# raviraina/grok

Measured on AMD Instinct MI355X. Metric: Mpixels/s encode+decode, 8K RGB 5/3 lossless + 9/7 lossy, 1/2/4/8 GPU, higher is better.
Workload: dtype int32 (5/3) + f32 (9/7)

## Files before the change

grok_amd/csrc/gk_engine.cpp:

```cpp
#include <hip/hip_runtime.h>

#include <algorithm>
#include <array>
#include <tuple>
#include <cmath>
#include <cstdarg>
#include <cstdlib>
#include <cstdio>
#include <cstring>
#include <memory>
#include <string>
#include <atomic>
#include <chrono>
#include <condition_variable>
#include <functional>
#include <mutex>
#include <thread>
#include <unordered_map>
#include <vector>
#include <queue>
#include <map>
#include <climits>
#include <linux/futex.h>
#include <sys/syscall.h>
// ... 3092 lines not shown
                    }
                    ctx->tm.dwt_launches++;
                    ctx->tm.dwt_bytes += area * (4 + es) * nc;
                    c += nc;
                }
                continue;
            }
            const GkComps cs{cst, ncr};
            if (irrev) {
                float* fs = reinterpret_cast<float*>(src_l);
                float* fd = reinterpret_cast<float*>(dst_l);
                if (forward) gk_launch_dwt97_fwd(ctx->st, fs, RG.stride, fd, RG.stride, w, h, S.tb, cs);
                else gk_launch_dwt97_inv(ctx->st, fd, RG.stride, fs, RG.stride, w, h, S.tb, cs);
            } else {
                if (forward) gk_launch_dwt53_fwd(ctx->st, src_l, RG.stride, dst_l, RG.stride, w, h, S.tb, cs);
                else gk_launch_dwt53_inv(ctx->st, dst_l, RG.stride, src_l, RG.stride, w, h, S.tb, cs);
            }
            ctx->tm.dwt_launches++;
            ctx->tm.dwt_bytes += area * 8 * ncr;
        }
    }
    }
}

static float ev_ms(gk_ctx* ctx, int a, int b) {
    float ms = 0; (void)hipEventElapsedTime(&ms, ctx->ev[a], ctx->ev[b]); return ms;
}

static void setup_plan(gk_ctx* ctx, const gk_image_info* info, const gk_cparameters* cp) {
    Plan want;
    want.w = info->w; want.h = info->h; want.nc = info->numcomps; want.prec = info->prec; want.sgnd = info->sgnd;
    set_params(want.p, cp, want.nc);
    want.x0 = info->x0; want.y0 = info->y0;
    want.gx0 = cp ? cp->tx0 : 0; want.gy0 = cp ? cp->ty0 : 0;
    if (!ctx->enc_dx.empty()) {
        if (ctx->enc_dx.size() != want.nc) throw GkError("gk_set_subsampling was given a different component count");
        want.cdx = ctx->enc_dx; want.cdy = ctx->enc_dy;
        if (!want.subsampled()) { want.cdx.clear(); want.cdy.clear(); }
    }
    if (want.gx0 > want.x0 || want.gy0 > want.y0) throw GkError("tile grid origin must lie at or above-left of the image origin");
    if ((uint64_t)want.x0 + want.w > 0xffffffffull || (uint64_t)want.y0 + want.h > 0xffffffffull)
        throw GkError("image area past the 32-bit canvas");
    if (want.p.tw && ((uint64_t)want.gx0 + want.p.tw <= want.x0 || (uint64_t)want.gy0 + want.p.th <= want.y0))
        throw GkError("the first tile must overlap the image area");
    if (want.nc < 3) want.p.mct = 0;
    if (ctx->enc_col.clears_mct()) want.p.mct = 0;
    if (want.p.mct && !want.mct3()) want.p.mct = 0;
    check_poc_coverage(want.p, want.nc);
    if ((want.p.cblk_sty & GK_STY_HT) && want.p.cblk_sty != GK_STY_HT)
        throw GkError("HTJ2K cannot be combined with Part-1 mode switches");
    if (want.p.cblk_sty > 0x7f) throw GkError("unknown code-block style bits");
    if (want.nc > 255 || want.nc == 0) throw GkError("bad component count");
    if (want.prec == 0 || want.prec > 31) throw GkError("component precision must be 1..31 bits");
    check_precision(want);
    if (want.w == 0 || want.h == 0) throw GkError("empty image");
    if (want.p.jp2) ctx->enc_jp2h = jp2h_content(want, &ctx->enc_col);
    if (want.p.cbw < 2 || want.p.cbh < 2 || want.p.cbw > 10 || want.p.cbh > 10 || want.p.cbw + want.p.cbh > 12)
        throw GkError("code-block size must be 4..1024 per side with at most 4096 samples");
    ensure_plan(ctx, want);
    restore_native_qcd(ctx);
    if (!ctx->plan.p.roishift.empty())
    for (const TileG& T : ctx->plan.tiles)
        for (uint32_t ci = 0; ci < (uint32_t)T.comps.size(); ++ci)
            for (const ResG& R : T.comps[ci].res)
                for (const auto& B : R.bands)
                    if (ctx->plan.p.roi(ci) && B.numbps > 25) throw GkError("ROI shift too large for this precision");
}

static void dump_blocks(gk_ctx* ctx, const uint32_t* hinfo, const GkPass* dps, uint32_t npass_total,
                        uint8_t* dbytes, uint64_t slot0) {
    const Plan& P = ctx->plan;
    hipStream_t st = ctx->st;
    const bool ht = P.p.ht();
    std::vector<GkPass> hp(std::max(npass_total, 1u));
    if (!ht && npass_total)
        HIPCHK(hipMemcpyAsync(hp.data(), dps, sizeof(GkPass) * npass_total, hipMemcpyDeviceToHost, st));
    HIPCHK(hipStreamSynchronize(st));
    ctx->rb_bands.clear(); ctx->rb_blocks.clear(); ctx->rb_passes.clear();
    std::vector<uint64_t> seg;
    uint64_t pos = 0;
    const TileG& T = P.tiles[0];
    for (uint32_t c = 0; c < P.nc; ++c)
        for (uint32_t r = 0; r < P.p.numres; ++r) {
            const ResG& R = T.comps[c].res[r];
            for (uint32_t bi = 0; bi < R.bands.size(); ++bi) {
                const BandG& B = R.bands[bi];
                ctx->rb_bands.push_back({c, r, bi, B.orient, R.pw * R.ph, B.step_enc});
                for (uint32_t pi = 0; pi < R.pw * R.ph; ++pi) {
                    const PrecG& PG = R.prc[bi][pi];
                    for (uint32_t k = 0; k < PG.cw * PG.ch; ++k) {
                        const uint32_t b = PG.first_block + k;
                        const GkBlock& G = P.blocks[b];
                        gk_block_result o{};
                        o.comp = c; o.res = r; o.band = bi; o.precinct = pi; o.cblk = k;
                        o.x0 = P.bxy[2 * (size_t)b]; o.y0 = P.bxy[2 * (size_t)b + 1];
                        o.x1 = o.x0 + G.w; o.y1 = o.y0 + G.h;
                        o.numbps = hinfo[4 * (size_t)b]; o.npasses = hinfo[4 * (size_t)b + 1];
                        o.len = hinfo[4 * (size_t)b + 2];
                        o.pass_off = (uint32_t)ctx->rb_passes.size();
                        o.data_off = pos;
                        const uint64_t so = G.data_off - slot0;
                        if (ht && o.npasses) {
                            const uint32_t ms = hinfo[4 * (size_t)b + 3], tl = o.len - ms;
                            if (ms) { seg.push_back(so); seg.push_back(pos); seg.push_back(ms); }
                            seg.push_back(so + G.data_cap - tl); seg.push_back(pos + ms); seg.push_back(tl);
                            ctx->rb_passes.push_back({o.len, o.len, 0.0});
                        } else if (o.npasses) {
                            seg.push_back(so); seg.push_back(pos); seg.push_back(o.len);
                            const GkPass* ps = hp.data() + hinfo[4 * (size_t)b + 3];
                            for (uint32_t q = 0; q < o.npasses; ++q)
                                ctx->rb_passes.push_back({q + 1 == o.npasses ? o.len : ps[q].rate, ps[q].len, ps[q].dist});
                        }
                        pos += o.len;
                        ctx->rb_blocks.push_back(o);
                    }
                }
            }
        }
    ctx->rb_data.resize(pos);
    if (pos) {
        uint64_t* hs = (uint64_t*)ctx->hseg.get(seg.size() * 8);
        memcpy(hs, seg.data(), seg.size() * 8);
        uint64_t* ds = (uint64_t*)ctx->dseg.get(seg.size() * 8);
        HIPCHK(hipMemcpyAsync(ds, hs, seg.size() * 8, hipMemcpyHostToDevice, st));
        uint8_t* dst = (uint8_t*)ctx->dout.get(pos);
        gk_launch_gather(st, dbytes, dst, ds, (uint32_t)(seg.size() / 3));
        HIPCHK(hipMemcpyAsync(ctx->rb_data.data(), dst, pos, hipMemcpyDeviceToHost, st));
        HIPCHK(hipStreamSynchronize(st));
    }
}

struct PixSrc { const void* pixels; size_t row_bytes; int on_device; };

static size_t encode_impl(gk_ctx* ctx, const gk_image_info* info, const void* const* comps, const uint32_t* strides,
                          int comps_on_device, const gk_cparameters* cp, uint8_t* out, size_t cap, int out_on_device,
                          int* rc, uint32_t tb = 0, uint32_t te = 0, bool with_header = true,
                          uint32_t* part_lens = nullptr, bool blocks_only = false, const PixSrc* pix = nullptr) {
    setup_plan(ctx, info, cp);
    Plan& P = ctx->plan;
    const uint32_t ntiles = (uint32_t)P.tiles.size();
    if (te == 0) { tb = 0; te = ntiles; }
    if (tb >= te || te > ntiles) throw GkError("bad tile range");
    const bool sub = P.subsampled();
    const uint32_t nb = (uint32_t)P.blocks.size();
    const uint32_t b0 = P.tiles[tb].b0, b1 = P.tiles[te - 1].b1, nbr = b1 - b0;
    const uint32_t jb = tb / P.ntx, je = (te - 1) / P.ntx + 1;
    const uint32_t ry0 = P.tiles[jb * P.ntx].y0 - P.y0, ry1 = P.tiles[(je - 1) * P.ntx].y1 - P.y0;
    hipStream_t st = ctx->st;

    launch_check(__LINE__);

    HIPCHK(hipEventRecord(ctx->ev[0], st));
    const Region RG = make_region(0, ry0, P.w, ry1);
    int32_t* arena = (int32_t*)ctx->arena.get(RG.plane * P.nc * 2 * sizeof(int32_t));
    const uint32_t nrows = ry1 - ry0;
    const int stype = sample_type(info->sample_bytes, P.prec, P.sgnd != 0);
    const size_t es = gk_sample_size(stype);
    std::vector<const void*> src(P.nc);
    std::vector<uint32_t> sstr(P.nc);
    std::vector<Region> RGg;
    for (const SGroup& G : P.groups) RGg.push_back(group_region(P, RG, G));
    if (pix) {
        const size_t tight = (size_t)RG.w * P.nc * es;
        const uint8_t* first = (const uint8_t*)pix->pixels + (size_t)RG.y0 * pix->row_bytes;
        GkUnpixArgs ua{};
        ua.ds = align_up(RG.w, GK_UNPIX_ALIGN);
        ua.plane = (uint64_t)ua.ds * RG.h;
        ua.w = RG.w; ua.h = RG.h; ua.nch = P.nc;
        ua.dst = ctx->dplanes.get(ua.plane * P.nc * es);
        ua.src = first; ua.row_bytes = pix->row_bytes;
        if (!pix->on_device) {
            void* dp = ctx->dpix_in.get(tight * RG.h);
            HIPCHK(hipMemcpy2DAsync(dp, tight, first, pix->row_bytes, tight, RG.h, hipMemcpyHostToDevice, st));
            ua.src = dp; ua.row_bytes = tight;
        }
        gk_launch_unpixels(st, (int)es, ua);
        for (uint32_t c = 0; c < P.nc; ++c) { src[c] = (const uint8_t*)ua.dst + (size_t)c * ua.plane * es; sstr[c] = ua.ds; }
    } else {
        size_t tot = 0;
        for (uint32_t c = 0; c < P.nc; ++c) tot += (size_t)RGg[P.group_of[c]].w * RGg[P.group_of[c]].h;
        uint8_t* dp = comps_on_device ? nullptr : (uint8_t*)ctx->dplanes.get(tot * es + 16);
        size_t o = 0;
        for (uint32_t c = 0; c < P.nc; ++c) {
            const Region& R = RGg[P.group_of[c]];
            const uint8_t* first = (const uint8_t*)comps[c] + (size_t)R.y0 * strides[c] * es;
            if (comps_on_device) { src[c] = first; sstr[c] = strides[c]; continue; }
            HIPCHK(hipMemcpy2DAsync(dp + o * es, (size_t)R.w * es, first, (size_t)strides[c] * es, (size_t)R.w * es, R.h,
                                    hipMemcpyHostToDevice, st));
            src[c] = dp + o * es; sstr[c] = R.w;
            o += (size_t)R.w * R.h;
        }
    }
    launch_check(__LINE__);
    HIPCHK(hipEventRecord(ctx->ev[1], st));
    int32_t shift = P.sgnd ? 0 : (1 << (P.prec - 1));
    auto planeA = [&](uint32_t c) { return arena + (size_t)c * 2 * RG.plane; };
    auto planeAf = [&](uint32_t c) { return reinterpret_cast<float*>(planeA(c)); };
    const bool mct3 = P.mct3();
    if (mct3 && (sstr[1] != sstr[0] || sstr[2] != sstr[0])) throw GkError("the first three components must share a stride");
    L1Io io;
    const bool fused = P.p.numres > 1 && P.l1_fusable;
    if (fused) {
        io.stype = stype; io.mct3 = mct3; io.shift.assign(P.nc, shift);
        io.planes.assign(src.begin(), src.end());
        io.strides = sstr;
    } else {
        auto cw = [&](uint32_t c) { return RGg[P.group_of[c]].w; };
        auto ch = [&](uint32_t c) { return RGg[P.group_of[c]].h; };
        if (!P.p.irrev) {
            if (mct3) gk_launch_dc_rct_fwd(st, stype, src[0], src[1], src[2], sstr[0], planeA(0), planeA(1), planeA(2), RG.stride, cw(0), ch(0), shift);
            for (uint32_t c = mct3 ? 3 : 0; c < P.nc; ++c) gk_launch_dc_fwd(st, stype, src[c], sstr[c], planeA(c), RG.stride, cw(c), ch(c), shift);
        } else {
            if (mct3) gk_launch_dc_ict_fwd(st, stype, src[0], src[1], src[2], sstr[0], planeAf(0), planeAf(1), planeAf(2), RG.stride, cw(0), ch(0), shift);
            for (uint32_t c = mct3 ? 3 : 0; c < P.nc; ++c) gk_launch_dc_fwd_f(st, stype, src[c], sstr[c], planeAf(c), RG.stride, cw(c), ch(c), shift);
        }
    }
    launch_check(__LINE__);
    HIPCHK(hipEventRecord(ctx->ev[2], st));
    run_dwt(ctx, RG, true, jb, je, 0, 0xffffffffu, fused ? &io : nullptr);
    if (const char* dp = getenv("GK_DUMP_DWT")) {
        std::vector<int32_t> hv((size_t)P.nc * 2 * RG.plane);
        HIPCHK(hipMemcpyAsync(hv.data(), arena, hv.size() * 4, hipMemcpyDeviceToHost, st));
        HIPCHK(hipStreamSynchronize(st));
        if (FILE* f = fopen(dp, "wb")) {
            const uint32_t hd[4] = {P.nc, RG.stride, RG.h, RG.w};
            fwrite(hd, 4, 4, f);
            fwrite(hv.data(), 4, hv.size(), f);
            fclose(f);
        }
    }
    launch_check(__LINE__);
    HIPCHK(hipEventRecord(ctx->ev[3], st));
    const bool do_rc = P.p.rate_control();
    const uint64_t slot0 = P.blocks[b0].data_off;
    const uint64_t slot1 = b1 < nb ? P.blocks[b1].data_off : P.slot_bytes;
    const uint64_t slot_span = slot1 - slot0;
    uint8_t* dbytes = (uint8_t*)ctx->bytes.get(slot_span + (64u << 20));
    const uint32_t nbx = std::max(nbr, 1u);
    GkBlock* dblk = (GkBlock*)ctx->dblocks.get(sizeof(GkBlock) * nbx);
    GkPass* dps = (GkPass*)ctx->dpasses.get(sizeof(GkPass) * GK_MAX_PASSES * (size_t)nbx);
    uint32_t* dinfo = (uint32_t*)ctx->dinfo.get(16 * (size_t)nbx + 16);
    int* derr = (int*)ctx->derr.get(64);
    uint32_t* dpcount = (uint32_t*)(derr + 4);
    uint8_t* dsym = P.p.ht() ? nullptr : (uint8_t*)ctx->dsym.get(P.sym_off[b1] - P.sym_off[b0] + 256);
    uint64_t* dsymoff = (uint64_t*)ctx->dsymoff.get(8 * ((size_t)nbr + 1));
    uint32_t* dpe = (uint32_t*)ctx->dpassend.get(4 * GK_MAX_PASSES * (size_t)nbx);
    uint32_t* dcm = (uint32_t*)ctx->dcminfo.get(8 * (size_t)nbx);
    int32_t* dnmse = do_rc ? (int32_t*)ctx->dnmse.get(4 * GK_MAX_PASSES * (size_t)nbx) : nullptr;
    if (!ctx->blocks_uploaded || ctx->enc_b0 != b0 || ctx->enc_b1 != b1 || ctx->enc_rc != do_rc) {
        GkBlock* hb = (GkBlock*)ctx->hpasses.get(sizeof(GkBlock) * nbx + 8 * ((size_t)nbr + 1));
        uint64_t* hso = (uint64_t*)(hb + nbx);
        for (uint32_t i = 0; i < nbr; ++i) {
            hb[i] = P.blocks[b0 + i];
            hb[i].band_off = relocate(P, group_region(P, RG, P.groups[P.group_of[hb[i].comp]]), hb[i].band_off);
            hb[i].stride = RG.stride;
            hb[i].data_off -= slot0;
            hb[i].flags = (uint8_t)((hb[i].flags & ~2u) | (do_rc ? 2u : 0u));
        }
        for (uint32_t i = 0; i <= nbr; ++i) hso[i] = P.sym_off[b0 + i] - P.sym_off[b0];
        HIPCHK(hipMemcpyAsync(dblk, hb, sizeof(GkBlock) * nbr, hipMemcpyHostToDevice, st));
        HIPCHK(hipMemcpyAsync(dsymoff, hso, 8 * ((size_t)nbr + 1), hipMemcpyHostToDevice, st));
        HIPCHK(hipStreamSynchronize(st));
        ctx->blocks_uploaded = true; ctx->enc_b0 = b0; ctx->enc_b1 = b1; ctx->enc_rc = do_rc;
    }
    HIPCHK(hipMemsetAsync(derr, 0, 64, st));
    const uint32_t nsolo_env = []() { const char* v = getenv("GK_T1ENC_SOLO"); return v ? (uint32_t)atoi(v) : 0u; }();
    if (P.p.ht()) {
        uint8_t* mel = (uint8_t*)ctx->dsym.get((size_t)nbx * GK_HT_MEL_CAP + 256);
        launch_check(__LINE__);
        HIPCHK(hipEventRecord(ctx->ev[8], st));
        gk_launch_ht_enc(st, arena, dblk, dbytes, mel, GK_HT_MEL_CAP, dinfo, nbr, derr, P.p.wide());
    } else if (P.p.t1_generic()) {
        uint8_t* mst = (uint8_t*)ctx->dmsstate.get(gk_t1ms_state_bytes(nbx));
        launch_check(__LINE__);
        HIPCHK(hipEventRecord(ctx->ev[8], st));
        gk_launch_t1_enc_ms(st, arena, dblk, dbytes, dps, dinfo, nbr, derr, ctx->nmse_tab, dpcount, mst, P.p.cblk_sty & 0x3f);
    } else if (nbr < 8192 || getenv("GK_T1ENC_SERIAL")) {
        gk_launch_t1_cm(st, arena, dblk, dsymoff, dsym, dpe, dcm, nbr, derr, ctx->nmse_tab, dnmse);
        launch_check(__LINE__);
        HIPCHK(hipEventRecord(ctx->ev[8], st));
        gk_launch_t1_mq(st, dsym, dsymoff, dpe, dcm, dblk, dbytes, dps, dinfo, nbr, derr, dnmse, dpcount, nullptr, 0,
                        0xffffffffu, std::min(nsolo_env, nbr));
    } else {
        uint32_t* dw = (uint32_t*)ctx->dweight.get(4 * (size_t)nbr);
        gk_launch_t1_weight(st, arena, dblk, dw, nbr);
        uint32_t* hw = (uint32_t*)ctx->hweight.get(4 * (size_t)nbr);
        HIPCHK(hipMemcpyAsync(hw, dw, 4 * (size_t)nbr, hipMemcpyDeviceToHost, st));
        HIPCHK(hipStreamSynchronize(st));
        uint32_t wmax = 1;
        for (uint32_t i = 0; i < nbr; ++i) wmax = std::max(wmax, hw[i]);
        const uint32_t kB = 4096;
        auto key = [&](uint32_t i) { return kB - 1 - (uint32_t)(((uint64_t)hw[i] * (kB - 1)) / wmax); };
        std::vector<uint32_t> start(kB + 1, 0);
        for (uint32_t i = 0; i < nbr; ++i) start[key(i)]++;
        for (uint32_t k = 0, acc = 0; k <= kB; ++k) { const uint32_t c = start[k]; start[k] = acc; acc += c; }
        uint32_t* ho = (uint32_t*)ctx->hord_enc.get(4 * (size_t)nbr);
        for (uint32_t i = 0; i < nbr; ++i) ho[start[key(i)]++] = i;
        uint32_t* dord = (uint32_t*)ctx->dord_enc.get(4 * (size_t)nbr);
        HIPCHK(hipMemcpyAsync(dord, ho, 4 * (size_t)nbr, hipMemcpyHostToDevice, st));
        static std::vector<double> frs[2];
        std::vector<double>& fr = frs[do_rc ? 1 : 0];
        if (fr.empty()) {
            const char* cv = getenv("GK_T1ENC_CUTS");
            std::string cs = cv ? cv : (do_rc ? "0.08,0.25" : "0.125,0.375");
            for (size_t q = 0; q < cs.size();) {
                size_t e = cs.find(',', q);
                if (e == std::string::npos) e = cs.size();
                const double f = atof(cs.substr(q, e - q).c_str());
                if (f > 0 && f < 1 && fr.size() < 3) fr.push_back(f);
                q = e + 1;
            }
        }
        std::vector<uint32_t> cut(1, 0);
        for (double f : fr) {
            const uint32_t c = (uint32_t)(nbr * f) / 256 * 256;
            if (c > cut.back() && c < nbr) cut.push_back(c);
        }
        cut.push_back(nbr);
        const int nch = (int)cut.size() - 1;
        for (int k = 0; k < nch; ++k) {
            const uint32_t base = cut[k], cnt = cut[k + 1] - cut[k];
            gk_launch_t1_cm(st, arena, dblk, dsymoff, dsym, dpe, dcm, nbr, derr, ctx->nmse_tab, dnmse, dord, base, cnt);
            if (k + 1 < nch) {
                HIPCHK(hipEventRecord(ctx->xev[k], st));
                HIPCHK(hipStreamWaitEvent(ctx->aux[k], ctx->xev[k], 0));
                gk_launch_t1_mq(ctx->aux[k], dsym, dsymoff, dpe, dcm, dblk, dbytes, dps, dinfo, nbr, derr, dnmse, dpcount,
                                dord, base, cnt, k == 0 ? std::min(nsolo_env, cnt) : 0u);
                HIPCHK(hipEventRecord(ctx->xev[3 + k], ctx->aux[k]));
            } else {
                launch_check(__LINE__);
                HIPCHK(hipEventRecord(ctx->ev[8], st));
                gk_launch_t1_mq(st, dsym, dsymoff, dpe, dcm, dblk, dbytes, dps, dinfo, nbr, derr, dnmse, dpcount, dord,
                                base, cnt);
            }
        }
        for (int k = 0; k + 1 < nch; ++k) HIPCHK(hipStreamWaitEvent(st, ctx->xev[3 + k], 0));
    }
    launch_check(__LINE__);
    HIPCHK(hipEventRecord(ctx->ev[4], st));
    static const bool eprof = getenv("GK_PROFILE") != nullptr;
    using eclk = std::chrono::steady_clock;
    auto ems = [](eclk::time_point a, eclk::time_point b) { return std::chrono::duration<double, std::milli>(b - a).count(); };
    const auto te0 = eclk::now();
    uint32_t* hinfo = (uint32_t*)ctx->hinfo.get(16 * (size_t)nb + 64);
    HIPCHK(hipMemcpyAsync(hinfo + 4 * (size_t)b0, dinfo, 16 * (size_t)nbr, hipMemcpyDeviceToHost, st));
    HIPCHK(hipMemcpyAsync(hinfo + 4 * (size_t)nb, derr, 32, hipMemcpyDeviceToHost, st));
    HIPCHK(hipStreamSynchronize(st));
    const uint32_t t1err = hinfo[4 * (size_t)nb], npass_total = hinfo[4 * (size_t)nb + 4];
    if (t1err) throw GkError(t1err & 2 ? "T1 symbol buffer overflow" : "T1 code-block slot overflow");
    const bool ht = P.p.ht();
    const GkPass* hpasses = nullptr;
    if ((do_rc || (P.p.cblk_sty & (GK_STY_LAZY | GK_STY_TERMALL))) && !ht) {
        GkPass* hp = (GkPass*)ctx->hpasses.get(sizeof(GkPass) * (size_t)std::max(npass_total, 1u));
        HIPCHK(hipMemcpyAsync(hp, dps, sizeof(GkPass) * (size_t)npass_total, hipMemcpyDeviceToHost, st));
        HIPCHK(hipStreamSynchronize(st));
        hpasses = hp;
    }
    if (blocks_only) {
        dump_blocks(ctx, hinfo, dps, npass_total, dbytes, slot0);
        *rc = 0;
        return 0;
    }

    std::vector<uint8_t> H;
    H.reserve(1 << 12);
    size_t tlm_pos = 0;
    write_main_header(H, P, &tlm_pos);
    const size_t rc_header_size = H.size() + (P.p.jp2 ? jp2_prefix_size(P, ctx->enc_jp2h) : 0);
    if (!with_header) H.clear();
    const auto te1 = eclk::now();
    if (const char* ds = getenv("GK_DUMP_SYMS"); ds && dsym && !P.p.t1_generic()) {
        std::vector<uint32_t> pe((size_t)GK_MAX_PASSES * nbr), cm(2 * (size_t)nbr), out(2 * (size_t)nbr);
        HIPCHK(hipMemcpy(pe.data(), dpe, 4 * pe.size(), hipMemcpyDeviceToHost));
        HIPCHK(hipMemcpy(cm.data(), dcm, 4 * cm.size(), hipMemcpyDeviceToHost));
        for (uint32_t i = 0; i < nbr; ++i) {
            out[2 * i] = cm[2 * i + 1] ? pe[(size_t)GK_MAX_PASSES * i + cm[2 * i + 1] - 1] : 0;
            out[2 * i + 1] = cm[2 * i];
        }
        if (FILE* f = fopen(ds, "wb")) { fwrite(out.data(), 4, out.size(), f); fclose(f); }
    }
    if (const char* dp = getenv("GK_DUMP_PASSES")) {
        if (FILE* f = fopen(dp, "wb")) {
            const uint32_t hdr[2] = {nb, npass_total};
            fwrite(hdr, 4, 2, f);
            fwrite(hinfo, 16, nb, f);
            if (hpasses) fwrite(hpasses, sizeof(GkPass), npass_total, f);
            fclose(f);
        }
    }
    T2Enc T2(P, hinfo, hpasses, tb, te);
    std::vector<T2Enc::Swallow> tsw(te - tb);
    if (te - tb == 1 || !P.p.rate_control()) {
        T2.allocate(rc_header_size);
        tsw[0] = T2.final_sw;
    } else {
        const bool par = te - tb >= host_pool().size();
        auto one = [&](size_t q) {
            const uint32_t t = tb + (uint32_t)q;
            T2Enc Tt(P, hinfo, hpasses, t, t + 1);
            Tt.serial = par;
            Tt.allocate(rc_header_size);
            tsw[q] = Tt.final_sw;
            const TileG& TG = P.tiles[t];
            std::copy(Tt.lnp.begin() + (size_t)TG.b0 * T2.L, Tt.lnp.begin() + (size_t)TG.b1 * T2.L,
                      T2.lnp.begin() + (size_t)TG.b0 * T2.L);
        };
        if (par) host_pool().run(te - tb, one);
        else for (uint32_t q = 0; q < te - tb; ++q) one(q);
    }
    const auto te2 = eclk::now();
    std::vector<uint64_t> seg;
    seg.reserve(3 * ((size_t)nb * (ht ? 2 : 1) + 64));
    std::vector<uint8_t> hdrs;
    uint64_t pos = 0;
    auto add_host = [&](const uint8_t* p, size_t n) {
        if (!n) return;
        seg.push_back(slot_span + hdrs.size()); seg.push_back(pos); seg.push_back(n);
        hdrs.insert(hdrs.end(), p, p + n);
        pos += n;
    };
    std::vector<uint8_t> J;
    const bool jp2 = P.p.jp2 && with_header;
    if (jp2) write_jp2_prefix(J, P, 0, ctx->enc_jp2h);
    add_host(J.data(), J.size());
    const size_t main_at = J.size();
    add_host(H.data(), H.size());
    struct Pk { uint32_t hoff, hlen, s0, s1, len; };
    struct TileOut {
        std::vector<uint8_t> tp;
        std::vector<uint8_t> phdr;
        std::vector<Pk> pk;
        std::vector<uint32_t> bsegs;
        uint64_t psot = 0;
        std::vector<uint32_t> pkey;
        std::vector<uint32_t> tp_off, pk_first;
        std::vector<uint64_t> psots;
    };
    const TilePartSplit TPS = tile_part_split(P);
    if (part_lens && TPS.n > 1) throw GkError("tile-part generation is not supported with tile sharding");
    std::vector<TileOut> tout(te - tb);
    const bool par_chains = te - tb == 1;
    auto build_tile_part = [&](uint32_t t, TileOut& O) {
        const TileG& T = P.tiles[t];
        const T2Enc::Swallow& sw = tsw[t - tb];
        struct Chain { uint32_t r, c, pi; };
        std::vector<Chain> chains;
        for (uint32_t r = 0; r < P.p.numres; ++r)
            for (uint32_t c = 0; c < P.nc; ++c)
                for (uint32_t pi = 0; pi < T.comps[c].res[r].pw * T.comps[c].res[r].ph; ++pi) chains.push_back({r, c, pi});
        const uint32_t L = P.p.nlayers;
        std::vector<TileOut> co(chains.size());
        auto run_chain = [&](size_t q) {
            const Chain& ch = chains[q];
            const ResG& R = T.comps[ch.c].res[ch.r];
            TileOut& C = co[q];
            std::vector<uint32_t> body;
            std::vector<uint8_t> hb;
            for (uint32_t l = 0; l < L; ++l) {
                body.clear();
                T2.write_packet(R, ch.pi, l, nullptr, &body, hb);
                Pk k{(uint32_t)C.phdr.size(), (uint32_t)hb.size(), (uint32_t)C.bsegs.size(), 0, (uint32_t)hb.size()};
                C.phdr.insert(C.phdr.end(), hb.begin(), hb.end());
                for (size_t i = 0; i < body.size(); i += 3) {
                    if (!body[i + 2]) continue;
                    C.bsegs.push_back(body[i]); C.bsegs.push_back(body[i + 1]); C.bsegs.push_back(body[i + 2]);
                    k.len += body[i + 2];
                }
                k.s1 = (uint32_t)C.bsegs.size();
                C.pk.push_back(k);
            }
        };
        if (par_chains && chains.size() > 1) {
            struct BandU { uint32_t q, bi; };
            std::vector<BandU> bu;
            std::vector<uint32_t> bu0(chains.size() + 1, 0);
            for (size_t q = 0; q < chains.size(); ++q) {
                const ResG& R = T.comps[chains[q].c].res[chains[q].r];
                for (uint32_t bi = 0; bi < R.bands.size(); ++bi)
                    if (R.prc[bi][chains[q].pi].cw && R.prc[bi][chains[q].pi].ch) bu.push_back({(uint32_t)q, bi});
                bu0[q + 1] = (uint32_t)bu.size();
            }
            std::vector<std::vector<RawBits>> ubit(bu.size(), std::vector<RawBits>(L));
            std::vector<std::vector<uint32_t>> useg(bu.size());
            std::vector<std::vector<uint32_t>> uend(bu.size(), std::vector<uint32_t>(L));
            std::vector<size_t> bord(bu.size());
            for (size_t i = 0; i < bord.size(); ++i) bord[i] = bord.size() - 1 - i;
            host_pool().run(bord.size(), [&](size_t j) {
                const size_t u = bord[j];
                const Chain& ch = chains[bu[u].q];
                const ResG& R = T.comps[ch.c].res[ch.r];
                const PrecG& PG = R.prc[bu[u].bi][ch.pi];
                T2.band_init(PG, R.bands[bu[u].bi].numbps);
                std::vector<uint32_t>& sg = useg[u];
                for (uint32_t l = 0; l < L; ++l) {
                    RawBits& rb = ubit[u][l];
                    T2.band_header(PG, l, rb);
                    rb.finish();
                    for (uint32_t k = 0; k < PG.cw * PG.ch; ++k) {
                        const uint32_t b = PG.first_block + k;
                        const uint32_t np = T2.lnp[(size_t)b * L + l];
                        if (!np) continue;
                        const uint32_t r0 = T2.inprev[b] ? T2.rate(b, T2.inprev[b] - 1) : 0, r1 = T2.rate(b, T2.inprev[b] + np - 1);
                        if (r1 > r0) { sg.push_back(b); sg.push_back(r0); sg.push_back(r1 - r0); }
                        T2.inprev[b] = (uint16_t)(T2.inprev[b] + np);
                    }
                    uend[u][l] = (uint32_t)sg.size();
                }
            });
            host_pool().run(chains.size(), [&](size_t q) {
                TileOut& C = co[q];
                for (uint32_t l = 0; l < L; ++l) {
                    const uint32_t h0 = (uint32_t)C.phdr.size();
                    PktBitWriter bw(C.phdr);
                    bw.putbit(1);
                    for (uint32_t u = bu0[q]; u < bu0[q + 1]; ++u) {
                        const RawBits& rb = ubit[u][l];
                        const size_t full = (size_t)(rb.n / 64);
                        const uint32_t rem = (uint32_t)(rb.n % 64);
                        for (size_t i = 0; i < full; ++i) { bw.put((uint32_t)(rb.w[i] >> 32), 32); bw.put((uint32_t)rb.w[i], 32); }
                        if (rem) {
                            const uint64_t x = rb.w[full] >> (64 - rem);
                            if (rem > 32) { bw.put((uint32_t)(x >> 32), rem - 32); bw.put((uint32_t)x, 32); }
                            else bw.put((uint32_t)x, rem);
                        }
                    }
                    bw.flush();
                    const uint32_t hlen = (uint32_t)C.phdr.size() - h0;
                    Pk k{h0, hlen, (uint32_t)C.bsegs.size(), 0, hlen};
                    for (uint32_t u = bu0[q]; u < bu0[q + 1]; ++u) {
                        const uint32_t s0 = l ? uend[u][l - 1] : 0, s1 = uend[u][l];
                        for (uint32_t i = s0; i < s1; i += 3) k.len += useg[u][i + 2];
                        C.bsegs.insert(C.bsegs.end(), useg[u].begin() + s0, useg[u].begin() + s1);
                    }
                    k.s1 = (uint32_t)C.bsegs.size();
                    C.pk.push_back(k);
                }
            });
        } else {
            for (size_t q = 0; q < chains.size(); ++q) run_chain(q);
        }
        std::vector<uint32_t> chain_at(P.p.numres * P.nc + 1, 0);
        for (uint32_t r = 0, q = 0; r < P.p.numres; ++r)
            for (uint32_t c = 0; c < P.nc; ++c) { chain_at[r * P.nc + c] = q; q += T.comps[c].res[r].pw * T.comps[c].res[r].ph; }
        std::vector<uint32_t> entry;
        const std::vector<PacketRef> order = packet_order(P, T, L, &P.p.pocs, TPS.poc ? &entry : nullptr);
        for (size_t oi = 0; oi < order.size(); ++oi) {
                const PacketRef& pr = order[oi];
                O.pkey.push_back(TPS.poc ? entry[2 * oi] : TPS.key(pr));
                const size_t q = chain_at[pr.r * P.nc + pr.c] + pr.pi;
                const uint32_t l = pr.l;
                const TileOut& C = co[q];
                Pk k = C.pk[l];
                const uint32_t h0 = (uint32_t)O.phdr.size(), s0 = (uint32_t)O.bsegs.size();
                if (P.p.sop_eph & 2) {
                    const uint32_t nsop = (TPS.poc ? entry[2 * oi + 1] : (uint32_t)O.pk.size()) & 0xffff;
                    const uint8_t sop[6] = {0xff, 0x91, 0, 4, (uint8_t)(nsop >> 8), (uint8_t)nsop};
                    O.phdr.insert(O.phdr.end(), sop, sop + 6);
                }
                O.phdr.insert(O.phdr.end(), C.phdr.begin() + k.hoff, C.phdr.begin() + k.hoff + k.hlen);
                if (P.p.sop_eph & 4) { O.phdr.push_back(0xff); O.phdr.push_back(0x92); }
                const uint32_t ovh = ((P.p.sop_eph & 2) ? 6 : 0) + ((P.p.sop_eph & 4) ? 2 : 0);
                k.hlen += ovh; k.len += ovh;
                O.bsegs.insert(O.bsegs.end(), C.bsegs.begin() + k.s0, C.bsegs.begin() + k.s1);
                k.hoff = h0; k.s1 = s0 + (k.s1 - k.s0); k.s0 = s0;
                O.pk.push_back(k);
            }
        std::vector<uint8_t>& tp = O.tp;
        size_t pk0 = 0;
        for (uint32_t part = 0; part < TPS.n; ++part) {
            size_t pk1 = pk0;
            while (pk1 < O.pk.size() && O.pkey[pk1] == part) ++pk1;
            const size_t h0 = tp.size();
            O.tp_off.push_back((uint32_t)h0); O.pk_first.push_back((uint32_t)pk0);
            put16(tp, 0xff90); put16(tp, 10); put16(tp, t); put32(tp, 0); tp.push_back((uint8_t)part);
            tp.push_back((uint8_t)TPS.n);
            if (part == 0 && !P.p.pocs.empty()) write_poc(tp, P.p.pocs, P.nc, &P, t == 0 ? P.p.prog : ~0u);
            if (P.p.plt && part == 0) {
                std::vector<uint32_t> lens;
                const uint32_t ovh = ((P.p.sop_eph & 2) ? 6 : 0) + ((P.p.sop_eph & 4) ? 2 : 0);
                for (const PacketRef& pr : packet_order(P, T, L)) {
                    uint32_t len = co[chain_at[pr.r * P.nc + pr.c] + pr.pi].pk[pr.l].len + ovh;
                    if (sw.on && pr.c == sw.c && pr.r == sw.r && pr.pi == sw.pi && pr.l == sw.l)
                        len = (uint32_t)(len + sw.hcnt - sw.hreal);
                    lens.push_back(len);
                }
                std::vector<uint8_t> v;
                for (const uint32_t len : lens) {
                    const int nbits = floorlog2(len) + 1, nbytes = (nbits + 6) / 7;
                    for (int q = nbytes - 1; q >= 0; --q) v.push_back((uint8_t)(((len >> (7 * q)) & 0x7F) | (q ? 0x80 : 0)));
                }
                if (3 + v.size() > 65535) throw GkError("PLT marker overflow (too many packets in one tile)");
                put16(tp, 0xff58); put16(tp, (uint32_t)(3 + v.size())); tp.push_back(0);
                tp.insert(tp.end(), v.begin(), v.end());
            }
            put16(tp, 0xff93);
            uint64_t psot = tp.size() - h0;
            for (size_t q = pk0; q < pk1; ++q) psot += O.pk[q].len;
            if (TPS.n == 1 && sw.on) psot = psot + sw.hcnt - sw.hreal;
            if (psot > 0xffffffffull) throw GkError("tile part exceeds 4 GiB");
            tp[h0 + 6] = (uint8_t)(psot >> 24); tp[h0 + 7] = (uint8_t)(psot >> 16); tp[h0 + 8] = (uint8_t)(psot >> 8);
            tp[h0 + 9] = (uint8_t)psot;
            O.psots.push_back(psot);
            pk0 = pk1;
        }
        if (pk0 != O.pk.size()) throw GkError("tile-part split out of packet order");
        O.tp_off.push_back((uint32_t)tp.size()); O.pk_first.push_back((uint32_t)pk0);
        O.psot = O.psots[0];
// ... 2501 lines not shown
```

grok_amd/csrc/gk_t1enc.hip:

```cpp
#include <hip/hip_runtime.h>
#include <stdint.h>
#include "gk_common.h"
#include "gk_t1_common.h"
#include <algorithm>
#include <type_traits>
#include <cstdlib>

#define SYM_PER_PLANE 11264u

__device__ __forceinline__ uint32_t win6(uint64_t col, uint32_t s) {
    return (uint32_t)((s ? (col >> (4 * s - 1)) : (col << 1)) & 63u);
}

__device__ __forceinline__ uint32_t lane_prev(uint32_t v) {
    return (uint32_t)__builtin_amdgcn_update_dpp(0, (int)v, 0x138, 0xf, 0xf, false);
}
__device__ __forceinline__ uint32_t lane_next(uint32_t v) {
    return (uint32_t)__builtin_amdgcn_update_dpp(0, (int)v, 0x130, 0xf, 0xf, false);
}
__device__ __forceinline__ uint32_t wave_excl_scan(uint32_t v, uint32_t& total) {
    int inc = (int)v;
    inc += __builtin_amdgcn_update_dpp(0, inc, 0x111, 0xf, 0xf, false);
    inc += __builtin_amdgcn_update_dpp(0, inc, 0x112, 0xf, 0xf, false);
    inc += __builtin_amdgcn_update_dpp(0, inc, 0x114, 0xf, 0xf, false);
    inc += __builtin_amdgcn_update_dpp(0, inc, 0x118, 0xf, 0xf, false);
    inc += __builtin_amdgcn_update_dpp(0, inc, 0x142, 0xa, 0xf, false);
    inc += __builtin_amdgcn_update_dpp(0, inc, 0x143, 0xc, 0xf, false);
    total = (uint32_t)__builtin_amdgcn_readlane(inc, 63);
    return (uint32_t)inc - v;
}

__device__ __forceinline__ uint32_t nb9(uint32_t L, uint32_t C, uint32_t R, int r) {
    return ((L >> r) & 7u) | (((C >> r) & 7u) << 3) | (((R >> r) & 7u) << 6);
}
__device__ __forceinline__ uint32_t sc8(uint32_t fs, uint32_t fn) { return (fs & 0xaau) | ((fn >> 1) & 0x55u); }
__host__ __device__ constexpr uint32_t zc_of_nb9(uint32_t i) {
    return (i & 1u) | (((i >> 3) & 1u) << 1) | (((i >> 6) & 1u) << 2) | (((i >> 1) & 1u) << 3) | (((i >> 4) & 1u) << 4) |
           (((i >> 7) & 1u) << 5) | (((i >> 2) & 1u) << 6) | (((i >> 5) & 1u) << 7) | (((i >> 8) & 1u) << 8);
}
__host__ __device__ constexpr uint32_t sc_of_sc8(uint32_t i) {
    return (i & 3u) | (((i >> 6) & 3u) << 2) | (((i >> 2) & 3u) << 4) | (((i >> 4) & 3u) << 6);
}
struct alignas(16) CmTabs {
    uint8_t zc[4][512];
    uint8_t sc[256];
};
constexpr CmTabs make_cm_tabs() {
    CmTabs t{};
    for (uint32_t o = 0; o < 4; ++o)
        for (uint32_t i = 0; i < 512; ++i) t.zc[o][i] = zc_rule(o, zc_of_nb9(i));
    for (uint32_t i = 0; i < 256; ++i) t.sc[i] = sc_rule(sc_of_sc8(i));
    return t;
}
__constant__ CmTabs c_cm_tabs = make_cm_tabs();

struct alignas(16) CmLds {
    uint8_t zc[512];
    uint8_t sc[256];
};
struct CmRcLds {
    int16_t nm[4][128];
};

__device__ __forceinline__ int32_t wave_sum(int32_t v) {
#pragma unroll
    for (int o = 32; o > 0; o >>= 1) v += __shfl_xor(v, o);
    return v;
}

template <bool RC>
__global__ __launch_bounds__(64) void k_t1_cm(const int32_t* __restrict__ coef, const GkBlock* __restrict__ blocks,
                                              const uint64_t* __restrict__ sym_off, uint8_t* __restrict__ sym,
                                              uint32_t* __restrict__ pass_end, uint32_t* __restrict__ cm_info,
                                              uint32_t nblocks, int* err, const int16_t* __restrict__ nmse_tab,
                                              int32_t* __restrict__ pass_nmse, const uint32_t* __restrict__ order,
                                              uint32_t base, uint32_t count) {
    __shared__ CmLds L;
    __shared__ typename std::conditional<RC, CmRcLds, char>::type R;
    if (blockIdx.x >= count) return;
    const uint32_t b = order ? order[base + blockIdx.x] : base + blockIdx.x;
    if (b >= nblocks) return;
    const int lane = threadIdx.x;
    const GkBlock B = blocks[b];
    const uint32_t w = B.w, h = B.h;
    reinterpret_cast<uint2*>(L.zc)[lane] = reinterpret_cast<const uint2*>(c_cm_tabs.zc[B.orient & 3])[lane];
    reinterpret_cast<uint32_t*>(L.sc)[lane] = reinterpret_cast<const uint32_t*>(c_cm_tabs.sc)[lane];
    const bool irrev = B.flags & 1;
    uint32_t m[64];
    uint64_t negcol = 0;
    uint32_t mx = 0;
#pragma unroll
    for (int y = 0; y < 64; ++y) {
        int32_t raw = 0;
        uint32_t a = 0;
        if (y < (int)h && lane < (int)w) {
            raw = coef[B.band_off + (size_t)y * B.stride + lane];
            if (irrev) a = (uint32_t)fabsf(rintf((__int_as_float(raw) / B.step) * 64.0f));
            else a = (uint32_t)(raw < 0 ? -raw : raw) * 64u;
        }
        m[y] = a;
        mx = a > mx ? a : mx;
        negcol |= (uint64_t)(raw < 0) << y;
    }
    if (const uint32_t rs = B.flags >> 3) {
        mx = 0;
#pragma unroll
        for (int y = 0; y < 64; ++y) {
            m[y] = ((m[y] >> 6) << (6 + rs)) | (m[y] & 63u);
            mx = m[y] > mx ? m[y] : mx;
        }
    }
    if constexpr (RC) {
        for (int i = lane; i < 512; i += 64) R.nm[i >> 7][i & 127] = nmse_tab[i];
    }
#pragma unroll
    for (int o = 32; o > 0; o >>= 1) { uint32_t t = __shfl_xor(mx, o); mx = t > mx ? t : mx; }
    uint32_t numbps = 0;
    if (mx) { uint32_t t = 32 - __clz(mx); numbps = t <= 6 ? 0 : t - 6; }
    __syncthreads();
    if (numbps == 0) {
        if (lane == 0) { cm_info[2 * b] = 0; cm_info[2 * b + 1] = 0; }
        return;
    }
    const uint64_t base_off = sym_off[b];
    const uint64_t cap = sym_off[b + 1] - base_off;
    if ((uint64_t)numbps * SYM_PER_PLANE > cap) {
        if (lane == 0) { atomicOr(err, 2); cm_info[2 * b] = 0; cm_info[2 * b + 1] = 0; }
        return;
    }
    uint8_t* S = sym + base_off;
    uint32_t* PE = pass_end + (size_t)b * GK_MAX_PASSES;
    const uint64_t validcol = (lane < (int)w) ? ((h >= 64) ? ~0ull : ((1ull << h) - 1)) : 0ull;
    const uint32_t nstripes = (h + 3) >> 2;
    uint64_t sig = 0, mu = 0;
    uint32_t pos = 0, passno = 0;
    int32_t acc = 0;
    auto nm_rows = [&](uint64_t mask, int t, int bp) __attribute__((always_inline)) {
        if constexpr (RC) {
            const int16_t* tab = R.nm[bp > 0 ? t : t + 1];
#pragma unroll
            for (int g = 0; g < 8; ++g) {
                const uint32_t gm = (uint32_t)(mask >> (8 * g)) & 0xffu;
                if (__any(gm != 0)) {
#pragma unroll
                    for (int k = 0; k < 8; ++k)
                        if ((gm >> k) & 1) acc += tab[(m[8 * g + k] >> bp) & 127];
                }
            }
        }
    };
    auto end_pass = [&]() {
        if (lane == 0) PE[passno] = pos;
        if constexpr (RC) {
            int32_t t = wave_sum(acc);
            if (lane == 0) pass_nmse[(size_t)b * GK_MAX_PASSES + passno] = t;
            acc = 0;
        }
        ++passno;
    };

    for (int bpno = (int)numbps - 1; bpno >= 0; --bpno) {
        uint64_t bitcol = 0;
#pragma unroll
        for (int y = 0; y < 64; ++y) bitcol |= (uint64_t)((m[y] >> (bpno + 6)) & 1u) << y;
        uint64_t vis = 0;
        const uint64_t sigPrev = sig;
        if (bpno != (int)numbps - 1) {
            for (uint32_t s = 0; s < nstripes; ++s) {
                const uint32_t sh = 4 * s;
                const uint32_t Wc = win6(sig, s), Nc = win6(negcol, s);
                uint32_t pk = Wc | (Nc << 6);
                const uint32_t pL = lane_prev(pk), pR = lane_next(pk);
                const uint32_t WL = pL & 63, NL = (pL >> 6) & 63, WR = pR & 63, NR = (pR >> 6) & 63;
                const uint32_t valid4 = (uint32_t)(validcol >> sh) & 15u;
                const uint32_t cand = ~(Wc >> 1) & valid4;
                const uint32_t bit4 = (uint32_t)(bitcol >> sh) & 15u;
                const uint32_t A = ((WL | (WL >> 1) | (WL >> 2)) | (WR | (WR >> 1) | (WR >> 2)) | Wc | (Wc >> 2)) & 15u;
                auto F = [&](uint32_t in, uint32_t& cd) -> uint32_t {
                    uint32_t x = A | ((in | (in << 1) | (in >> 1)) & 15u);
                    uint32_t c0 = cand & x & 1u, n0 = c0 & bit4;
                    uint32_t c1 = cand & (x | (n0 << 1)) & 2u, n1 = c1 & bit4;
                    uint32_t c2 = cand & (x | (n1 << 1)) & 4u, n2 = c2 & bit4;
                    uint32_t c3 = cand & (x | (n2 << 1)) & 8u, n3 = c3 & bit4;
                    cd = c0 | c1 | c2 | c3;
                    return n0 | n1 | n2 | n3;
                };
                uint32_t cd, in = 0;
                uint32_t ns = F(0, cd);
                while (true) {
                    in = lane_prev(ns);
                    uint32_t cd2, ns2 = F(in, cd2);
                    bool ch = ns2 != ns;
                    ns = ns2; cd = cd2;
                    if (!__any(ch)) break;
                }
                const uint32_t Lt = WL | (in << 1), Cn = ns << 1;
                uint32_t cnt = __popc(cd) + __popc(ns);
                uint32_t total, off = wave_excl_scan(cnt, total);
                uint8_t* o = S + pos + off;
#pragma unroll
                for (int r = 0; r < 4; ++r) {
                    if ((cd >> r) & 1) {
                        const uint32_t d = (bit4 >> r) & 1;
                        const uint32_t fs = nb9(Lt, Wc | (Cn & ((2u << r) - 1)), WR, r);
                        *o++ = (uint8_t)(((CTX_ZC + L.zc[fs]) << 1) | d);
                        if (d) {
                            const uint32_t e = L.sc[sc8(fs, nb9(NL, Nc, NR, r))];
                            const uint32_t sg = (Nc >> (r + 1)) & 1;
                            *o++ = (uint8_t)(((CTX_SC + (e & 15)) << 1) | (sg ^ (e >> 4)));
                        }
                    }
                }
                pos += total;
                sig |= (uint64_t)ns << sh;
                vis |= (uint64_t)cd << sh;
            }
            nm_rows(sig & ~sigPrev, 0, bpno);
            end_pass();
            for (uint32_t s = 0; s < nstripes; ++s) {
                const uint32_t sh = 4 * s;
                const uint32_t Wc = win6(sig, s);
                const uint32_t pL = lane_prev(Wc), pR = lane_next(Wc);
                const uint32_t nb = ((pL | (pL >> 1) | (pL >> 2)) | (pR | (pR >> 1) | (pR >> 2)) | Wc | (Wc >> 2)) & 15u;
                const uint32_t mr = (uint32_t)(sigPrev >> sh) & 15u;
                const uint32_t mu4 = (uint32_t)(mu >> sh) & 15u;
                const uint32_t bit4 = (uint32_t)(bitcol >> sh) & 15u;
                uint32_t total, off = wave_excl_scan(__popc(mr), total);
                uint8_t* o = S + pos + off;
#pragma unroll
                for (int r = 0; r < 4; ++r) {
                    if ((mr >> r) & 1) {
                        uint32_t cx = ((mu4 >> r) & 1) ? CTX_MAG + 2 : (((nb >> r) & 1) ? CTX_MAG + 1 : CTX_MAG);
                        *o++ = (uint8_t)((cx << 1) | ((bit4 >> r) & 1));
                    }
                }
                pos += total;
            }
            nm_rows(sigPrev, 2, bpno);
            mu |= sigPrev;
            end_pass();
        }
        const uint64_t sigCu = sig;
        for (uint32_t s = 0; s < nstripes; ++s) {
            const uint32_t sh = 4 * s;
            const uint32_t Wc = win6(sig, s), Nc = win6(negcol, s);
            const uint32_t valid4 = (uint32_t)(validcol >> sh) & 15u;
            const uint32_t vis4 = (uint32_t)(vis >> sh) & 15u;
            const uint32_t bit4 = (uint32_t)(bitcol >> sh) & 15u;
            const uint32_t cl = ~(Wc >> 1) & ~vis4 & valid4;
            const uint32_t nc = cl & bit4;
            uint32_t pk = Wc | (Nc << 6) | (nc << 12);
            const uint32_t pL = lane_prev(pk), pR = lane_next(pk);
            const uint32_t WL = pL & 63, NL = (pL >> 6) & 63, ncL = (pL >> 12) & 15;
            const uint32_t WR = pR & 63, NR = (pR >> 6) & 63;
            const uint32_t Lt = WL | (ncL << 1), Cn = nc << 1;
            const bool agg = (valid4 == 15u) && (cl == 15u) && ((Lt | WR | (Wc & 0x21u)) == 0);
            uint32_t rl = nc ? (uint32_t)__ffs(nc) - 1 : 4u;
            uint32_t cnt;
            uint32_t codemask;
            if (agg) {
                if (rl == 4) { cnt = 1; codemask = 0; }
                else {
                    codemask = cl & ~((2u << rl) - 1);
                    cnt = 3 + 1 + __popc(codemask) + __popc(nc & codemask);
                }
            } else {
                codemask = cl;
                cnt = __popc(cl) + __popc(nc);
            }
            uint32_t total, off = wave_excl_scan(cnt, total);
            uint8_t* o = S + pos + off;
            if (agg) {
                *o++ = (uint8_t)((CTX_AGG << 1) | (rl != 4 ? 1 : 0));
                if (rl != 4) {
                    *o++ = (uint8_t)((CTX_UNI << 1) | (rl >> 1));
                    *o++ = (uint8_t)((CTX_UNI << 1) | (rl & 1));
                    const uint32_t sg = (Nc >> (rl + 1)) & 1;
                    *o++ = (uint8_t)((CTX_SC << 1) | sg);
                }
            }
#pragma unroll
            for (int r = 0; r < 4; ++r) {
                if ((codemask >> r) & 1) {
                    const uint32_t d = (bit4 >> r) & 1;
                    const uint32_t fs = nb9(Lt, Wc | (Cn & ((2u << r) - 1)), WR, r);
                    *o++ = (uint8_t)(((CTX_ZC + L.zc[fs]) << 1) | d);
                    if (d) {
                        const uint32_t e = L.sc[sc8(fs, nb9(NL, Nc, NR, r))];
                        const uint32_t sg = (Nc >> (r + 1)) & 1;
                        *o++ = (uint8_t)(((CTX_SC + (e & 15)) << 1) | (sg ^ (e >> 4)));
                    }
                }
            }
            pos += total;
            sig |= (uint64_t)nc << sh;
        }
        nm_rows(sig & ~sigCu, 0, bpno);
        end_pass();
    }
    if (lane == 0) { cm_info[2 * b] = numbps; cm_info[2 * b + 1] = passno; }
}

#define MQ_RING_DW 32
struct MqLane {
    uint32_t a, c, ct;
    int32_t bp;
    uint32_t cur;
    uint8_t* out;
    uint32_t cap;
    uint32_t lf;
    uint32_t pcx1, pne1, epref;
};
struct MqLds {
    uint32_t tab[96];
    uint32_t ctx[20][64];
    uint32_t ring[64][MQ_RING_DW + 1];
};

__device__ __forceinline__ void mq_line_store(MqLane& q, MqLds& L, int lane, uint32_t li) {
    const uint32_t o = (li & 1) * 16;
    uint8_t* dst = q.out + (size_t)li * 64;
    if ((li + 1) * 64 <= q.cap) {
#pragma unroll
        for (int i = 0; i < 4; ++i)
            *(uint4*)(dst + 16 * i) = make_uint4(L.ring[lane][o + 4 * i], L.ring[lane][o + 4 * i + 1],
                                                 L.ring[lane][o + 4 * i + 2], L.ring[lane][o + 4 * i + 3]);
    } else {
        for (uint32_t i = 0; i < 16 && li * 64 + 4 * i + 4 <= q.cap; ++i) *(uint32_t*)(dst + 4 * i) = L.ring[lane][o + i];
    }
}
__device__ __forceinline__ void mq_lines_out(MqLane& q, MqLds& L, int lane) {
    const uint32_t cl = (uint32_t)max(q.bp, 0) >> 6;
    if (__any(cl > q.lf)) {
        if (cl > q.lf) { mq_line_store(q, L, lane, q.lf); q.lf++; }
    }
}

__device__ __forceinline__ void mq_put5(MqLane& q, MqLds& L, int lane, uint32_t bo, uint32_t cur) {
    uint8_t* row = reinterpret_cast<uint8_t*>(&L.ring[lane][0]);
    row[(uint32_t)q.bp & (4 * MQ_RING_DW - 1)] = (uint8_t)cur;
    q.bp -= (int32_t)bo;
}
template <bool CARRY = true>
__device__ __forceinline__ void mq_byteout5(MqLane& q, MqLds& L, int lane, uint32_t bo, uint32_t& c, uint32_t& ct) {
    uint32_t cur = q.cur;
    if constexpr (CARRY) {
        const uint32_t carry = (c >> 27) & 1u & bo & ~mz(q.cur ^ 0xffu);
        cur += carry;
        c &= ~(carry << 27);
    }
    const uint32_t ffm = mz(cur ^ 0xffu);
    const uint32_t nb = __builtin_amdgcn_ubfe(c, 19u - ffm, 8);
    mq_put5(q, L, lane, bo, cur);
    q.cur = bsel(bo, nb, q.cur);
    c &= (0x7ffffu | (ffm & 0x80000u)) | ~bo;
    ct = bsel(bo, 8u + ffm, ct);
}

#define MQ_CT_PARKED (1u << 30)
__device__ __forceinline__ void mq_code5(MqLane& q, MqLds& L, int lane, uint32_t s, uint32_t s_next) {
    const uint32_t cx = min(s >> 1, 19u);
    const uint32_t e = bsel(mz(opq(cx ^ q.pcx1)), q.pne1, q.epref);
    L.ctx[q.pcx1][lane] = q.pne1;
    q.epref = L.ctx[min(s_next >> 1, 19u)][lane];
    const uint32_t mpsm = mneg(e), qe = e & 0xffff;
    const uint32_t a1 = q.a - qe;
    const uint32_t ism = ~(mpsm ^ mbit(s, 0));
    const uint32_t fast = ism & mbit(a1, 15);
    const uint32_t x = ism ^ mlt(a1, qe);
    uint32_t nidx;
    asm("v_bfi_b32 %0, %1, %2, %3" : "=v"(nidx) : "v"(ism), "v"(__builtin_amdgcn_ubfe(e, 16, 7)), "v"(__builtin_amdgcn_ubfe(e, 23, 7)));
    const uint32_t ne = L.tab[nidx];
    q.pcx1 = cx; q.pne1 = bsel(fast, e, ne);
    const uint32_t an = bsel(x, a1, qe);
    const uint32_t n = ffbh(an) - 16u;
    q.a = an << n;
    uint32_t c = q.c + (qe & x);
    const uint32_t n1 = min(n, q.ct);
    uint32_t n2 = n - n1;
    const bool two = __any(n2 >= 7u);
    c <<= n1;
    uint32_t ct = q.ct - n1;
    mq_byteout5(q, L, lane, mz(ct), c, ct);
    if (two) {
        const uint32_t n2a = min(n2, ct);
        c <<= n2a; ct -= n2a; n2 -= n2a;
        mq_byteout5<false>(q, L, lane, mz(ct), c, ct);
    }
    q.c = c << n2;
    q.ct = ct - n2;
}

__device__ __forceinline__ uint32_t byte_of(uint4 v, uint32_t j) {
    const uint32_t w = j < 4 ? v.x : j < 8 ? v.y : j < 12 ? v.z : v.w;
    return (w >> (8 * (j & 3))) & 0xff;
}

__device__ __forceinline__ uint32_t srl(uint32_t v, uint32_t lane) {
    return (uint32_t)__builtin_amdgcn_readlane((int)v, (int)lane);
}
__device__ __forceinline__ uint32_t swl(uint32_t old, uint32_t val, uint32_t lane) {
    asm("v_writelane_b32 %0, %1, m0" : "+v"(old) : "s"(val), "{m0}"(lane));
    return old;
}
struct MqSolo {
    uint32_t a, c, ct;
    int32_t bp;
    uint32_t cur;
    uint32_t wacc;
    uint32_t ring;
    __device__ __forceinline__ void byteout() {
        const bool ff = cur == 0xffu;
        const bool carry = !ff && (c & 0x8000000u);
        const uint32_t cur2 = cur + (carry ? 1u : 0u);
        const bool seven = cur2 == 0xffu;
        const uint32_t cc = carry ? c & 0x7ffffffu : c;
        const uint32_t nb = seven ? (cc >> 20) & 0xffu : (cc >> 19) & 0xffu;
        wacc |= cur2 << (8u * ((uint32_t)bp & 3u));
        ring = swl(ring, wacc, ((uint32_t)bp >> 2) & 63u);
        ++bp;
        wacc = ((uint32_t)bp & 3u) ? wacc : 0u;
        cur = nb;
        c = seven ? cc & 0xfffffu : cc & 0x7ffffu;
        ct = seven ? 7u : 8u;
    }
};

__device__ void mq_solo_block(uint32_t b, const uint8_t* __restrict__ sym, const uint64_t* __restrict__ sym_off,
                              const uint32_t* __restrict__ pass_end, const uint32_t* __restrict__ cm_info,
                              const GkBlock* __restrict__ blocks, uint8_t* __restrict__ bytes,
                              GkPass* __restrict__ passes, uint32_t* __restrict__ info, int* err,
                              const int32_t* __restrict__ pass_nmse, uint32_t* __restrict__ pass_counter, int lane) {
    const uint32_t numbps = cm_info[2 * b], npasses = cm_info[2 * b + 1];
    if (npasses == 0) {
        if (lane == 0) { info[4 * b] = 0; info[4 * b + 1] = 0; info[4 * b + 2] = 0; info[4 * b + 3] = 0; }
        return;
    }
    const uint32_t* PE = pass_end + (size_t)b * GK_MAX_PASSES;
    const uint32_t nsym = PE[npasses - 1];
    const GkBlock B = blocks[b];
    const uint8_t* sp = sym + sym_off[b];
    uint8_t* out = bytes + B.data_off;
    const uint32_t cap = B.data_cap;
    uint32_t poff = 0;
    if (lane == 0) poff = atomicAdd(pass_counter, npasses);
    poff = srl(poff, 0);
    GkPass* P = passes + poff;
    const bool rc = (B.flags & 2) != 0;
    double cum = 0.0;
    const uint32_t TAB0 = mq_pair_entry((uint32_t)lane), TAB1 = lane < MQ_PAIRS - 64 ? mq_pair_entry(64u + lane) : 0u;
    uint32_t CTX = mq_pair_entry(2u * (lane == CTX_ZC ? 4u : (lane == CTX_AGG ? 3u : (lane == CTX_UNI ? 46u : 0u))));
    MqSolo q;
    q.a = 0x8000; q.c = 0; q.ct = 12; q.bp = -1; q.cur = 0; q.wacc = 0; q.ring = 0;
    uint32_t lf = 0;
    auto lines_out = [&](uint32_t upto) {
        for (; lf < upto; ++lf)
            if ((uint32_t)(lane >> 4) == (lf & 3u) && lf * 64 + 64 <= cap)
                *reinterpret_cast<uint32_t*>(out + (size_t)lf * 64 + 4 * (lane & 15)) = q.ring;
    };
    auto chunk = [&](uint32_t k) -> uint32_t {
        return (lane < 16 && 64 * k < nsym) ? *reinterpret_cast<const uint32_t*>(sp + 64 * k + 4 * lane) : 0u;
    };
    uint32_t p = 0, next_end = PE[0];
    auto close_pass = [&]() {
        uint32_t rate;
        if (p == npasses - 1) {
            const uint32_t tempc = q.c + q.a;
            q.c |= 0xffffu;
            if (q.c >= tempc) q.c -= 0x8000u;
            q.c <<= q.ct; q.byteout();
            q.c <<= q.ct; q.byteout();
            if (q.cur != 0xffu) {
                q.wacc |= q.cur << (8u * ((uint32_t)q.bp & 3u));
                q.ring = swl(q.ring, q.wacc, ((uint32_t)q.bp >> 2) & 63u);
                ++q.bp;
            }
            rate = (uint32_t)q.bp;
        } else {
            rate = (uint32_t)q.bp + 5u + (q.ct < 5 ? 1u : 0u);
        }
        if (rc) {
            const int bpno = p == 0 ? (int)numbps - 1 : (int)numbps - 2 - (int)(p - 1) / 3;
            double wm = __dmul_rn(B.wmse, (double)(1 << bpno));
            wm = __dmul_rn(wm, __dmul_rn(wm, (double)pass_nmse[(size_t)b * GK_MAX_PASSES + p]) / 8192.0);
            cum = __dadd_rn(cum, wm);
        }
        if (lane == 0) { P[p].rate = rate; P[p].dist = cum; }
        ++p;
        next_end = p < npasses ? PE[p] : 0xffffffffu;
    };
    while (p < npasses && next_end == 0) close_pass();
    uint32_t NX = chunk(0);
    for (uint32_t k = 0; 64 * k < nsym; ++k) {
        const uint32_t CH = NX;
        NX = chunk(k + 1);
        const uint32_t i1 = min(64 * k + 64, nsym);
        for (uint32_t i = 64 * k; i < i1; ++i) {
            const uint32_t s = (srl(CH, (i >> 2) & 15u) >> (8u * (i & 3u))) & 0xffu;
            const uint32_t cx = s >> 1;
            const uint32_t e = srl(CTX, cx);
            const uint32_t qe = e & 0xffffu;
            const uint32_t a1 = q.a - qe;
            const bool ism = (s & 1u) == (e >> 31);
            const bool x = ism != (a1 < qe);
            const bool fast = ism && (a1 & 0x8000u);
            const uint32_t nidx = ism ? (e >> 16) & 0x7fu : (e >> 23) & 0x7fu;
            const uint32_t t0 = srl(TAB0, nidx & 63u), t1 = srl(TAB1, nidx & 63u);
            CTX = swl(CTX, fast ? e : ((nidx & 64u) ? t1 : t0), cx);
            const uint32_t an = x ? a1 : qe;
            q.c += x ? qe : 0u;
            uint32_t n = (uint32_t)__builtin_clz(an) - 16u;
            q.a = an << n;
            if (n >= q.ct) {
                q.c <<= q.ct; n -= q.ct; q.byteout();
                if (n >= q.ct) { q.c <<= q.ct; n -= q.ct; q.byteout(); }
            }
            q.c <<= n; q.ct -= n;
            if (i + 1 == next_end)
                do close_pass(); while (p < npasses && next_end == i + 1);
        }
        lines_out((uint32_t)max(q.bp, 0) >> 6);
    }
    const uint32_t nbytes = (uint32_t)q.bp;
    if (lf * 64 < nbytes && (uint32_t)(lane >> 4) == (lf & 3u) && lf * 64 + 4 * (lane & 15) + 4 <= cap &&
        (uint32_t)(lane & 15) * 4 < nbytes - lf * 64)
        *reinterpret_cast<uint32_t*>(out + (size_t)lf * 64 + 4 * (lane & 15)) = q.ring;
    __threadfence();
    if (lane != 0) return;
    uint32_t last = nbytes;
    for (int k = (int)npasses; k > 0;) {
        GkPass& ps = P[--k];
        if (ps.rate > last) ps.rate = last; else last = ps.rate;
    }
    uint32_t prev = 0;
    for (uint32_t k = 0; k < npasses; ++k) {
        GkPass& ps = P[k];
        if (ps.rate > 0 && ps.rate <= cap && out[ps.rate - 1] == 0xff) ps.rate--;
        ps.len = ps.rate - prev;
        prev = ps.rate;
    }
    info[4 * b] = numbps;
    info[4 * b + 1] = npasses;
    info[4 * b + 2] = P[npasses - 1].rate;
    info[4 * b + 3] = poff;
    if (nbytes > cap) atomicOr(err, 1);
}

__global__ __launch_bounds__(256) void k_t1_mq(const uint8_t* __restrict__ sym, const uint64_t* __restrict__ sym_off,
                                              const uint32_t* __restrict__ pass_end, const uint32_t* __restrict__ cm_info,
                                              const GkBlock* __restrict__ blocks, uint8_t* __restrict__ bytes,
                                              GkPass* __restrict__ passes, uint32_t* __restrict__ info,
                                              uint32_t nblocks, int* err, const int32_t* __restrict__ pass_nmse,
                                              uint32_t* __restrict__ pass_counter, uint32_t nl,
// ... 206 lines not shown
```

Measured before the change: 1750.

## Batch coefficient loads, branchless NMSE accumulation, skip empty stripes in T1 encoder

The T1 code-block encoder now loads all coefficients in clamped, branch-free groups of eight rows before converting them, so the loads can be issued together. The NMSE accumulation becomes a masked, branchless sum. Each coding pass skips stripes where no lane has work, using wave-wide any votes. The default rate-control chunk cut points also move, which changes how blocks are split across launches. The clamped loads read a few redundant elements, and the extra any votes add some overhead on dense stripes.

```diff
diff --git a/grok_amd/csrc/gk_engine.cpp b/grok_amd/csrc/gk_engine.cpp
--- a/grok_amd/csrc/gk_engine.cpp
+++ b/grok_amd/csrc/gk_engine.cpp
@@ -3418,7 +3418,7 @@
         std::vector<double>& fr = frs[do_rc ? 1 : 0];
         if (fr.empty()) {
             const char* cv = getenv("GK_T1ENC_CUTS");
-            std::string cs = cv ? cv : (do_rc ? "0.08,0.25" : "0.125,0.375");
+            std::string cs = cv ? cv : (do_rc ? "0.05,0.15" : "0.125,0.375");
             for (size_t q = 0; q < cs.size();) {
                 size_t e = cs.find(',', q);
                 if (e == std::string::npos) e = cs.size();
diff --git a/grok_amd/csrc/gk_t1enc.hip b/grok_amd/csrc/gk_t1enc.hip
--- a/grok_amd/csrc/gk_t1enc.hip
+++ b/grok_amd/csrc/gk_t1enc.hip
@@ -89,15 +89,28 @@
     uint32_t m[64];
     uint64_t negcol = 0;
     uint32_t mx = 0;
+    if (w == 0 || h == 0) {
+        if (lane == 0) { cm_info[2 * b] = 0; cm_info[2 * b + 1] = 0; }
+        return;
+    }
+    const int32_t* src = coef + B.band_off + min((uint32_t)lane, w - 1);
+#pragma unroll
+    for (int g = 0; g < 8; ++g) {
+        if (8 * g < (int)h) {
+#pragma unroll
+            for (int y = 8 * g; y < 8 * g + 8; ++y) m[y] = (uint32_t)src[(size_t)min((uint32_t)y, h - 1) * B.stride];
+        } else {
+#pragma unroll
+            for (int y = 8 * g; y < 8 * g + 8; ++y) m[y] = 0;
+        }
+    }
 #pragma unroll
     for (int y = 0; y < 64; ++y) {
-        int32_t raw = 0;
-        uint32_t a = 0;
-        if (y < (int)h && lane < (int)w) {
-            raw = coef[B.band_off + (size_t)y * B.stride + lane];
-            if (irrev) a = (uint32_t)fabsf(rintf((__int_as_float(raw) / B.step) * 64.0f));
-            else a = (uint32_t)(raw < 0 ? -raw : raw) * 64u;
-        }
+        const bool in = y < (int)h && lane < (int)w;
+        const int32_t raw = in ? (int32_t)m[y] : 0;
+        uint32_t a;
+        if (irrev) a = (uint32_t)fabsf(rintf((__int_as_float(raw) / B.step) * 64.0f));
+        else a = (uint32_t)(raw < 0 ? -raw : raw) * 64u;
         m[y] = a;
         mx = a > mx ? a : mx;
         negcol |= (uint64_t)(raw < 0) << y;
@@ -142,9 +155,11 @@
             for (int g = 0; g < 8; ++g) {
                 const uint32_t gm = (uint32_t)(mask >> (8 * g)) & 0xffu;
                 if (__any(gm != 0)) {
-#pragma unroll
-                    for (int k = 0; k < 8; ++k)
-                        if ((gm >> k) & 1) acc += tab[(m[8 * g + k] >> bp) & 127];
+                    int32_t v[8];
+#pragma unroll
+                    for (int k = 0; k < 8; ++k) v[k] = tab[(m[8 * g + k] >> bp) & 127];
+#pragma unroll
+                    for (int k = 0; k < 8; ++k) acc += v[k] & (0 - (int32_t)((gm >> k) & 1u));
                 }
             }
         }
@@ -187,6 +202,7 @@
                 };
                 uint32_t cd, in = 0;
                 uint32_t ns = F(0, cd);
+                if (!__any(cd != 0)) continue;
                 while (true) {
                     in = lane_prev(ns);
                     uint32_t cd2, ns2 = F(in, cd2);
@@ -219,10 +235,11 @@
             end_pass();
             for (uint32_t s = 0; s < nstripes; ++s) {
                 const uint32_t sh = 4 * s;
+                const uint32_t mr = (uint32_t)(sigPrev >> sh) & 15u;
+                if (!__any(mr != 0)) continue;
                 const uint32_t Wc = win6(sig, s);
                 const uint32_t pL = lane_prev(Wc), pR = lane_next(Wc);
                 const uint32_t nb = ((pL | (pL >> 1) | (pL >> 2)) | (pR | (pR >> 1) | (pR >> 2)) | Wc | (Wc >> 2)) & 15u;
-                const uint32_t mr = (uint32_t)(sigPrev >> sh) & 15u;
                 const uint32_t mu4 = (uint32_t)(mu >> sh) & 15u;
                 const uint32_t bit4 = (uint32_t)(bitcol >> sh) & 15u;
                 uint32_t total, off = wave_excl_scan(__popc(mr), total);
@@ -249,6 +266,7 @@
             const uint32_t bit4 = (uint32_t)(bitcol >> sh) & 15u;
             const uint32_t cl = ~(Wc >> 1) & ~vis4 & valid4;
             const uint32_t nc = cl & bit4;
+            if (!__any(cl != 0)) continue;
             uint32_t pk = Wc | (Nc << 6) | (nc << 12);
             const uint32_t pL = lane_prev(pk), pR = lane_next(pk);
             const uint32_t WL = pL & 63, NL = (pL >> 6) & 63, ncL = (pL >> 12) & 15;
```

Result: faster. 1772, median of 6 (+1.3%).
